# ultralytics/yolov3

Measured on AMD Instinct MI355X. Metric: images/sec (640x640) inference+NMS, higher is better.
Workload: dtype f16; 1 GPU; yolov3 inference 640x640 batch=32/GPU fp16 nc=80 + NMS(conf 0.001, iou 0.6, multi_label, max_det 300) [BASELINE configs[1]]; global_batch=32, parallelism=replicas x1 (no data-path collective)

## Files before the change

include/yolov3_hip.h:

```cpp
#ifndef YOLOV3_HIP_H
#define YOLOV3_HIP_H

#include <stddef.h>
#include <stdint.h>

#ifdef __cplusplus
extern "C" {
#endif

#define Y3_ABI_VERSION 6

typedef enum { Y3_F16 = 0, Y3_BF16 = 1, Y3_F32 = 2, Y3_U8 = 3 } y3_dtype;
typedef enum { Y3_ACT_NONE = 0, Y3_ACT_SILU = 1 } y3_act;
typedef enum { Y3_ALGO_AUTO = 0, Y3_ALGO_MFMA = 1, Y3_ALGO_DIRECT = 2 } y3_algo;

typedef struct {
    void* data;
    int32_t n, h, w, c;
    int32_t pitch;
} y3_tensor;

typedef struct {
    int32_t dtype;
    int32_t ksize;
// ... 27 lines not shown
int y3_conv2d_fwd_variant(const y3_conv_desc* desc, const y3_tensor* x, const y3_tensor* y, int32_t has_residual,
                          size_t workspace_bytes, char* name, size_t name_capacity);
int y3_conv_v10_tiles(const y3_conv_desc* desc, const y3_tensor* x, const y3_tensor* y, size_t workspace_bytes, int32_t* records,
                      int64_t capacity, int64_t* n_tiles, int32_t* column_blocks, int32_t* group_blocks);
int64_t y3_conv2d_fwd_bnin_rows(const y3_conv_desc* desc, const y3_tensor* u_in, const y3_tensor* y_in, const y3_tensor* y, int32_t has_shortcut);
int y3_conv2d_fwd_bnin_stats(const y3_conv_desc* desc, const y3_tensor* u_in, const float* in_scale, const float* in_shift, int32_t in_act,
                             const y3_tensor* in_shortcut , const y3_tensor* y_in, const void* packed_filter, const float* bias, const y3_tensor* y,
                             float* stat_rows, int64_t capacity_rows, int64_t* n_rows, void* stream);
int y3_conv_last_variant(char* name, size_t name_cap);

size_t y3_packed_filter_stem_elems(int32_t cout);
int y3_pack_filter_stem(const float* w_oihw, int32_t cout_src, int32_t cin_src, int32_t cout, int32_t dtype, void* packed, void* stream);
int y3_stem_conv_fwd(const void* x_nchw, int32_t src_dtype, int32_t n, int32_t cin, int32_t h, int32_t w, float divisor, const void* packed,
                     const float* bias, int32_t dtype, int32_t act, const y3_tensor* y, void* stream);
int64_t y3_stem_conv_stats_rows(int32_t n, int32_t h, int32_t w);
int y3_stem_conv_fwd_stats(const void* x_nchw, int32_t src_dtype, int32_t n, int32_t cin, int32_t h, int32_t w, float divisor, const void* packed,
                           const float* bias, int32_t dtype, int32_t act, const y3_tensor* y, float* stat_rows, int64_t capacity_rows, int64_t* n_rows,
                           void* stream);
int y3_stem_pair_fwd(const void* x_nchw, int32_t src_dtype, int32_t n, int32_t cin, int32_t h, int32_t w, float divisor,
                     const void* packed0, const float* bias0, int32_t act0, const void* packed1, const float* bias1, int32_t act1,
                     int32_t dtype, const y3_tensor* y, void* stream);
int y3_bneck_pair_fwd(const y3_tensor* x, const void* packed1, const float* bias1, int32_t act1, const void* packed2, const float* bias2,
                      int32_t act2, int32_t add_residual, int32_t dtype, const y3_tensor* y, void* stream);

int y3_nchw_to_nhwc(const void* src, int32_t src_dtype, int32_t n, int32_t c, int32_t h, int32_t w, float divisor,
                    int32_t out_dtype, const y3_tensor* out, void* stream);
int y3_nhwc_to_nchw(const y3_tensor* src, int32_t dtype, void* dst, void* stream);

int y3_maxpool2d(const y3_tensor* x, const y3_tensor* y, int32_t dtype, int32_t k, int32_t stride, int32_t pad,
                 int32_t zpad_r, int32_t zpad_b, void* stream);
int y3_spp_pyramid(const y3_tensor* x, const y3_tensor* y3c , int32_t dtype,
                   void* stream);
int y3_upsample2x(const y3_tensor* x, const y3_tensor* y, int32_t dtype, void* stream);
int y3_copy_slice(const y3_tensor* x, const y3_tensor* y, int32_t dtype, void* stream);

int y3_detect_decode(const y3_tensor* head, int32_t dtype, int32_t na, int32_t no, const float* anchors_px,
                     float stride, void* raw, void* z, int64_t row_offset, int64_t total_rows, void* stream);
int y3_detect_decode_levels(const y3_tensor* heads, int32_t n_levels, int32_t dtype, int32_t na, int32_t no,
                            const float* anchors_px, const float* strides, void* const* raws, void* z,
                            const int64_t* row_offsets, int64_t total_rows, void* stream);

typedef struct {
    double iou_thres;
    float conf_thres;
    int32_t multi_label, agnostic;
    int32_t max_det, max_nms;
// ... 269 lines not shown
```

yolov3_amd/csrc/api.cpp:

```cpp
#include <atomic>
#include <mutex>
#include <stdarg.h>
#include <stdio.h>
#include <stdlib.h>
#include <string.h>

#include "../../include/yolov3_hip.h"
#include "y3_knobs.h"

static thread_local char g_err[512] = "";

void y3_set_error(const char* fmt, ...) {
    va_list ap;
    va_start(ap, fmt);
    vsnprintf(g_err, sizeof(g_err), fmt, ap);
    va_end(ap);
}

extern "C" const char* y3_last_error(void) { return g_err; }
extern "C" int y3_abi_version(void) { return Y3_ABI_VERSION; }

namespace {
struct Knob {
    const char* name;
    long long def;
};
const Knob kKnobs[] = {
    {"conv", 0}, {"conv_ahead", 3}, {"bn_nt_bytes", 64ll << 20},
    {"wgrad", 0}, {"wgrad_xcd", 2}, {"dgrad_quad", 1}, {"spp_direct", 0}, {"wgrad_strip", 1}, {"conv_strip", 1},
    {"conv_v10", 1}, {"v10_mp", 0}, {"v10_blocks", 0}, {"v10_half", 2}, {"v10_ksplit", 1}, {"v10_slices", 0},
    {"v10_group", 1}, {"tile_xcd", 1}, {"conv_1x1s", 1}, {"wgrad_patch", 1}, {"wgrad_blocks", 512}, {"nms_sort", 1},
    {"decode_tile", 1}, {"nms_head", 1216},
};
constexpr int kCount = (int)(sizeof(kKnobs) / sizeof(kKnobs[0]));
static_assert(kCount == Y3K_COUNT, "kKnobs and y3_knob_id (y3_common.h) list the same knobs in the same order");
std::atomic<long long> g_val[kCount];
std::once_flag g_once;

int knob_index(const char* key) {
    for (int i = 0; i < kCount; ++i)
        if (key && !strcmp(key, kKnobs[i].name)) return i;
    return -1;
}
void load_defaults() {
    for (int i = 0; i < kCount; ++i) g_val[i].store(kKnobs[i].def, std::memory_order_relaxed);
    const char* e = getenv("Y3_TUNE");
    if (!e) return;
    char buf[512];
    strncpy(buf, e, sizeof(buf) - 1);
    buf[sizeof(buf) - 1] = 0;
    for (char* tok = strtok(buf, ",;"); tok; tok = strtok(nullptr, ",;")) {
        char* eq = strchr(tok, '=');
        if (!eq) continue;
        *eq = 0;
        const int i = knob_index(tok);
// ... 37 lines not shown
```

yolov3_amd/csrc/stem.hip:

```cpp
#include "../../include/yolov3_hip.h"
#include "y3_common.h"

#include <hip/hip_runtime.h>
#include <stdint.h>
#include <type_traits>
#include <utility>

namespace {

struct StemArgs {
    const void* x;
    const void* w;
    const float* bias;
    void* y;
    int N, Cin, H, W;
    int ypitch, Cout;
    int act;
    int tiles_w, tiles_h;
    float divisor;
    float* stats;
};

constexpr int TR = 8, TW = 64;
constexpr int PR = TR + 2;
// ... 128 lines not shown
        }
        __builtin_amdgcn_fence(__ATOMIC_RELEASE, "wavefront");
        __builtin_amdgcn_wave_barrier();
    }
    if (want_stats) {
#pragma unroll
        for (int off = CH; off < 64; off <<= 1)
#pragma unroll
            for (int q = 0; q < 8; ++q) { st0[q] += __shfl_xor(st0[q], off, 64); st1[q] += __shfl_xor(st1[q], off, 64); }
        __syncthreads();
        float* red = (float*)patch;
        if (rp == 0) {
#pragma unroll
            for (int q = 0; q < 8; ++q) { red[(wv * CH + ch) * 16 + 2 * q] = st0[q]; red[(wv * CH + ch) * 16 + 2 * q + 1] = st1[q]; }
        }
        __syncthreads();
        if (tid < CH * 16 && (tid >> 4) * 8 + 8 <= p.Cout) {
            const float v = red[tid] + red[CH * 16 + tid] + red[2 * CH * 16 + tid] + red[3 * CH * 16 + tid];
            p.stats[(long long)blockIdx.x * p.Cout * 2 + tid] = v;
        }
    }
}

struct PairArgs {
    const void* x;
    const void* w0;
    const float* b0;
    const void* w1;
    const float* b1;
    void* y;
    int N, Cin, H, W, Ho, Wo, ypitch, act0, act1, kpad1;
    int tiles_w, tiles_h, n_tiles;
    int xcd;
    float divisor;
#ifdef Y3_TIMELINE
    unsigned long long* tl;
#endif
};
#ifdef Y3_TIMELINE
static unsigned long long* g_pair_tl = nullptr;
#define SP_T(i) do { asm volatile("s_waitcnt lgkmcnt(0)" ::: "memory"); const unsigned long long t_ = __builtin_amdgcn_s_memtime(); asm volatile("s_waitcnt lgkmcnt(0)" ::: "memory"); tsum[i] += t_ - tprev; tprev = t_; } while (0)
#else
#define SP_T(i) do { } while (0)
#endif
constexpr int QR = 4, QW = 32;
constexpr int R0 = 2 * QR + 1, C0 = 2 * QW + 1;
constexpr int XR = R0 + 2, XW = C0 + 3;
constexpr int L0E = C0 / 2 + 1, L0ROW = C0 * 64;

template <typename T, typename S>
__global__ __launch_bounds__(256, 2) void stem_pair_kernel(const PairArgs p) {
    typedef typename Mfma16<T>::frag frag;
    typedef T vec4 __attribute__((ext_vector_type(4)));
    typedef unsigned u32x4 __attribute__((ext_vector_type(4)));
    constexpr int PATCH_BYTES = XR * XW * 8, SLICE_BYTES = 4 * 32 * 64;
// ... 20 lines not shown
#pragma unroll
    for (int j = 0; j < NPX; ++j) {
        const int e = tid + j * 256;
        const int pr = e / XW;
        prc[j] = e < XR * XW ? (pr << 8) | (e - pr * XW) : -1;
    }
    constexpr int NT0 = (R0 * C0 + 31) / 32, NJ0 = (NT0 + 3) / 4;
    int l0rd[NJ0], l0wr[NJ0], l0rc[NJ0];
#pragma unroll
    for (int j = 0; j < NJ0; ++j) {
        int q = (wv + 4 * j) * 32 + frow;
        const bool live = q < R0 * C0;
        if (!live) q = R0 * C0 - 1;
        const int r = q / C0, c = q - r * C0, ci = c >> 1;
        l0rd[j] = (r * XW + c + 2 * fk) * 8;
        l0wr[j] = live ? r * L0ROW + ((c & 1) ? L0E * 64 : 0) + ci * 64 + ((fk ^ ((ci >> 2) & 3)) << 4) : -1;
        l0rc[j] = (r << 8) | c;
    }
    const int hw = p.H * p.W;

    T* __restrict__ yg = (T*)p.y;
    S raw[NPX][4];
    bool rin[NPX];
    auto fetch = [&](int tile) {
        int b = tile;
        const int tw = b % p.tiles_w; b /= p.tiles_w;
        const int th = b % p.tiles_h;
        const int n = b / p.tiles_h;
        const int gh0 = 2 * th * QR - 2, gw0 = 2 * tw * QW - 2;
        const S* __restrict__ xs = (const S*)p.x + (long long)n * p.Cin * hw;
#pragma unroll
        for (int j = 0; j < NPX; ++j) {
            const int gh = gh0 + (prc[j] >> 8), gw = gw0 + (prc[j] & 255);
            rin[j] = prc[j] >= 0 && (unsigned)gh < (unsigned)p.H && (unsigned)gw < (unsigned)p.W;
            if (rin[j]) {
                const unsigned o = (unsigned)(gh * p.W + gw);
#pragma unroll
                for (int c = 0; c < 4; ++c)
                    if (c < p.Cin) raw[j][c] = xs[o + (unsigned)(c * hw)];
            }
        }
    };
    const bool plain = std::is_same<S, T>::value && p.divisor == 1.0f;
    auto stash = [&]() {
#pragma unroll
        for (int j = 0; j < NPX; ++j) {
            const int e = tid + j * 256;
            if (e < XR * XW) {
                vec4 v = {(T)0.0f, (T)0.0f, (T)0.0f, (T)0.0f};
                if (rin[j]) {
                    bool done = false;
                    if constexpr (std::is_same<S, T>::value) {
                        if (plain) {
#pragma unroll
                            for (int c = 0; c < 4; ++c)
                                if (c < p.Cin) v[c] = raw[j][c];
                            done = true;
                        }
                    }
                    if (!done) {
#pragma unroll
                        for (int c = 0; c < 4; ++c)
                            if (c < p.Cin) v[c] = from_f32<T>(src_f32<S>(raw[j][c]) / p.divisor);
                    }
                }
                *(vec4*)(scratch + e * 8) = v;
            }
        }
    };
    const int first = p.xcd ? xcd_remap((int)blockIdx.x, (int)gridDim.x) : (int)blockIdx.x;
    if (first < p.n_tiles) fetch(first);
#ifdef Y3_TIMELINE
    unsigned long long tsum[8] = {0, 0, 0, 0, 0, 0, 0, 0};
    unsigned long long tprev = __builtin_amdgcn_s_memtime();
#endif
    for (int tile = first; tile < p.n_tiles; tile += gridDim.x) {
        int b = tile;
        const int tw = b % p.tiles_w; b /= p.tiles_w;
        const int th = b % p.tiles_h;
        const int n = b / p.tiles_h;
        const int oh0 = th * QR, ow0 = tw * QW;
        const int gh0 = 2 * oh0 - 1, gw0 = 2 * ow0 - 1;
        const bool border = gh0 < 0 || gw0 < 0 || gh0 + R0 > p.H || gw0 + C0 > p.W;

        stash();
        SP_T(0);
        __syncthreads();
        SP_T(1);

#pragma unroll
        for (int j = 0; j < NJ0; ++j) {
            if (wv + 4 * j >= NT0) break;
            f32x16 acc;
#pragma unroll
            for (int g = 0; g < 4; ++g)
#pragma unroll
                for (int e = 0; e < 4; ++e) acc[4 * g + e] = cb0[8 * g + 4 * fk + e];
#pragma unroll
            for (int kh = 0; kh < 3; ++kh) {
                const unsigned char* src = scratch + l0rd[j] + kh * (XW * 8);
                typedef unsigned long long u64x2 __attribute__((ext_vector_type(2)));
                u64x2 rw;
                rw[0] = *(const unsigned long long*)src;
                rw[1] = *(const unsigned long long*)(src + 8);
                acc = Mfma16<T>::run(*(const frag*)(cw0 + ((frow * 3 + kh) * 16 + fk * 8) * 2), __builtin_bit_cast(frag, rw), acc);
            }
            if (p.act0 == Y3_ACT_SILU) silu_vec<f32x16, 16>(acc);
            bool keep = l0wr[j] >= 0;
            bool inside = true;
            if (border) inside = (unsigned)(gh0 + (l0rc[j] >> 8)) < (unsigned)p.H && (unsigned)(gw0 + (l0rc[j] & 255)) < (unsigned)p.W;
#pragma unroll
            for (int gp = 0; gp < 2; ++gp) {
                u32x4 ov;
#pragma unroll
                for (int h = 0; h < 2; ++h) {
                    const unsigned a = pack2<T>(acc[8 * gp + 2 * h], acc[8 * gp + 2 * h + 1]);
                    const unsigned b = pack2<T>(acc[8 * gp + 4 + 2 * h], acc[8 * gp + 4 + 2 * h + 1]);
                    const auto sw = __builtin_amdgcn_permlane32_swap(a, b, false, false);
                    ov[h] = inside ? (unsigned)sw[0] : 0u;
                    ov[2 + h] = inside ? (unsigned)sw[1] : 0u;
                }
                if (keep) *(u32x4*)(l0buf + (l0wr[j] ^ (gp << 5))) = ov;
            }
        }
        SP_T(2);
        __syncthreads();
        SP_T(3);
        if (tile + (int)gridDim.x < p.n_tiles) fetch(tile + gridDim.x);

        f32x16 acc1[2];
#pragma unroll
        for (int b2 = 0; b2 < 2; ++b2)
#pragma unroll
            for (int g = 0; g < 4; ++g)
#pragma unroll
                for (int e = 0; e < 4; ++e) acc1[b2][4 * g + e] = cb1[wc * 32 + 8 * g + 4 * fk + e];
#pragma unroll
        for (int tap = 0; tap < 9; ++tap) {
            const int kh = tap / 3, kw = tap - 3 * (tap / 3);
#pragma unroll
            for (int ks = 0; ks < 2; ++ks)
#pragma unroll
                for (int b2 = 0; b2 < 2; ++b2) {
                    const int lr = 2 * wp + b2;
                    const int ci = frow + (kw >> 1);
                    const frag bf = *(const frag*)(l0buf + (2 * lr + kh) * L0ROW + ((kw & 1) ? L0E * 64 : 0) + ci * 64 + (((ks * 2 + fk) ^ ((ci >> 2) & 3)) << 4));
                    acc1[b2] = Mfma16<T>::run(a1f[tap * 2 + ks], bf, acc1[b2]);
                }
        }
        SP_T(4);
        unsigned char* wl = scratch + wv * (32 * 64);
// ... 32 lines not shown
            __builtin_amdgcn_fence(__ATOMIC_RELEASE, "wavefront");
            __builtin_amdgcn_wave_barrier();
        }
        SP_T(5);
        __syncthreads();
        SP_T(6);
    }
#ifdef Y3_TIMELINE
    if (p.tl && blockIdx.x < 64 && lane == 0) {
#pragma unroll
        for (int i = 0; i < 8; ++i) p.tl[(blockIdx.x * 4 + wv) * 8 + i] = tsum[i];
    }
#endif
}

struct BneckArgs {
    const void* x;
    const void* w1;
    const float* b1;
    const void* w2;
    const float* b2;
    void* y;
    int N, H, W, xpitch, ypitch, act1, act2, add, kpad1, kpad2;
    int tiles_w, tiles_h, n_tiles;
    int xcd;
    unsigned x_bytes;
};
constexpr int BC = 32, RC = BC + 2;
constexpr int bneck_rows(int c) { return c == 64 ? 8 : 4; }
constexpr int L1PITCH = 40;

template <typename F, int... Is> Y3_DEV void sfor_impl(F&& f, std::integer_sequence<int, Is...>) { (f(std::integral_constant<int, Is>{}), ...); }
template <int N, typename F> Y3_DEV void sfor(F&& f) { sfor_impl(f, std::make_integer_sequence<int, N>{}); }

template <typename T, int C>
__global__ __launch_bounds__(C * 4, C == 64 ? 2 : 1) void bneck_pair_kernel(const BneckArgs p) {
    typedef typename Mfma16<T>::frag frag;
    typedef unsigned u32x4 __attribute__((ext_vector_type(4)));
    typedef __attribute__((address_space(3))) void* lds_ptr_t;
    constexpr int BR = bneck_rows(C), RW = BR / 2;
    constexpr int RR = BR + 2, RPX = RR * RC;
    constexpr int NT1 = (RPX + 31) / 32;
    constexpr int CM = C / 2;
    constexpr int FT = C / 32;
    constexpr int NWV = 2 * FT;
    constexpr int XB = C * 2, XCHK = XB / 16;
    constexpr int LB = CM * 2, LCHK = LB / 16;
    constexpr int K1S = C / 16, M1 = CM / 32;
    constexpr int KT = CM / 16;
    constexpr int K2S = 9 * KT;
    constexpr int XPIECES = (RPX * XCHK + 63) / 64;
    constexpr int XJ = (XPIECES + NWV - 1) / NWV;
    constexpr int NJ1 = (NT1 + NWV - 1) / NWV;
    constexpr int QSTEP = 32 * NWV;
    constexpr int XKS = XCHK == 8 ? 1 : 0;
    constexpr int LKS = LCHK == 4 ? 2 : 1;
    __shared__ __attribute__((aligned(16))) unsigned char xbuf[XPIECES * 1024];
    __shared__ __attribute__((aligned(16))) unsigned char l1buf[RR * L1PITCH * LB];
    __shared__ __attribute__((aligned(16))) unsigned char slices[NWV * 32 * 64];
    __shared__ __attribute__((aligned(16))) float cb1[CM], cb2[C];
    constexpr bool W1_LDS = C == 128;
    __shared__ __attribute__((aligned(16))) unsigned char cw1[W1_LDS ? CM * C * 2 : 16];

    const int tid = threadIdx.x, lane = tid & 63;
    const int wv = __builtin_amdgcn_readfirstlane(tid >> 6);
    const int frow = lane & 31, fk = lane >> 5;
    const int wc = wv >> 1, wp = wv & 1;

    if (tid < CM / 4) ((f32x4*)cb1)[tid] = ((const f32x4*)p.b1)[tid];
    else if (tid < CM / 4 + C / 4) ((f32x4*)cb2)[tid - CM / 4] = ((const f32x4*)p.b2)[tid - CM / 4];
    if constexpr (W1_LDS) {
        for (int i = tid; i < CM * XCHK; i += 64 * NWV) {
            const int r = i / XCHK, c = i % XCHK;
            *(u32x4*)(cw1 + r * XB + ((c ^ (r & 15)) << 4)) = *(const u32x4*)((const T*)p.w1 + (long long)r * p.kpad1 + c * 8);
        }
    }
    frag a2f[K2S];
#pragma unroll
    for (int t = 0; t < K2S; ++t) a2f[t] = *(const frag*)((const T*)p.w2 + (long long)(wc * 32 + frow) * p.kpad2 + t * 16 + fk * 8);

    const auto rs_x = __builtin_amdgcn_make_buffer_rsrc((void*)p.x, 0, (int)p.x_bytes, 0x00020000);
    const int c1q0 = 32 * wv + frow;
    const int c1r0 = c1q0 / RC, c1c0 = c1q0 - c1r0 * RC;
    const int c1rd0 = c1q0 * XB + ((fk ^ ((c1q0 >> XKS) & (XCHK - 1))) << 4);
    int c2rd[3];
#pragma unroll
    for (int kw = 0; kw < 3; ++kw) c2rd[kw] = (frow + kw) * LB + ((fk ^ (((frow + kw) >> LKS) & (LCHK - 1))) << 4);

    T* __restrict__ yg = (T*)p.y;
    auto fetch = [&](int tile) {
        int b = tile;
        const int tw = b % p.tiles_w; b /= p.tiles_w;
        const int th = b % p.tiles_h;
        const int n = b / p.tiles_h;
        const int gh0 = th * BR - 1, gw0 = tw * BC - 1;
        int lane_f = lane;
        asm volatile("" : "+v"(lane_f));
        const int xq0 = (64 / XCHK) * wv + lane_f / XCHK;
        const unsigned xsrc = (unsigned)(((lane_f % XCHK) ^ ((xq0 >> XKS) & (XCHK - 1))) * 16);
        int r = 0, c = xq0;
#pragma unroll
        for (int j = 0; j < XJ; ++j) {
            if (wv + NWV * j >= XPIECES) break;
            const int gh = gh0 + r, gw = gw0 + c;
            const bool ok = xq0 + 32 * j < RPX && (unsigned)gh < (unsigned)p.H && (unsigned)gw < (unsigned)p.W;
            const unsigned off = ok ? (unsigned)(((n * p.H + gh) * p.W + gw) * p.xpitch) * 2u + xsrc : 0xffffffffu;
            const unsigned ldsa = __builtin_amdgcn_readfirstlane((unsigned)(uintptr_t)(lds_ptr_t)xbuf + (unsigned)((wv + NWV * j) * 1024));
            asm volatile("s_mov_b32 m0, %0\n\ts_nop 0\n\tbuffer_load_dwordx4 %1, %2, 0 offen lds" : : "s"(ldsa), "v"(off), "s"(rs_x) : "memory");
            c += 32;
            if (c >= RC) { c -= RC; r += 1; }
        }
    };
    const int first = p.xcd ? xcd_remap((int)blockIdx.x, (int)gridDim.x) : (int)blockIdx.x;
    if (first < p.n_tiles) fetch(first);
    for (int tile = first; tile < p.n_tiles; tile += gridDim.x) {
        int b = tile;
        const int tw = b % p.tiles_w; b /= p.tiles_w;
        const int th = b % p.tiles_h;
        const int n = b / p.tiles_h;
        const int oh0 = th * BR, ow0 = tw * BC;
        const int gh0 = oh0 - 1, gw0 = ow0 - 1;
        const bool border = gh0 < 0 || gw0 < 0 || gh0 + RR > p.H || gw0 + RC > p.W;

        frag a1g[W1_LDS ? 1 : K1S * M1];
        if constexpr (!W1_LDS) {
#pragma unroll
            for (int ks = 0; ks < K1S; ++ks)
#pragma unroll
                for (int m = 0; m < M1; ++m) a1g[ks * M1 + m] = *(const frag*)((const T*)p.w1 + (long long)(m * 32 + frow) * p.kpad1 + ks * 16 + fk * 8);
        }
        __builtin_amdgcn_s_waitcnt(0x0F70);
        __syncthreads();

        {
            f32x16 acc[NJ1][M1];
#pragma unroll
            for (int j = 0; j < NJ1; ++j)
#pragma unroll
                for (int m = 0; m < M1; ++m)
#pragma unroll
                    for (int g = 0; g < 4; ++g)
#pragma unroll
                        for (int e = 0; e < 4; ++e) acc[j][m][4 * g + e] = cb1[m * 32 + 8 * g + 4 * fk + e];
#pragma unroll
            for (int ks = 0; ks < K1S; ++ks) {
                frag af[M1];
#pragma unroll
                for (int m = 0; m < M1; ++m) {
                    if constexpr (W1_LDS) af[m] = *(const frag*)(cw1 + (m * 32 + frow) * XB + (((2 * ks + fk) ^ (frow & 15)) << 4));
                    else af[m] = a1g[ks * M1 + m];
                }
#pragma unroll
                for (int j = 0; j < NJ1; ++j) {
                    if (wv + NWV * j >= NT1) break;
                    const frag bf = *(const frag*)(xbuf + ((c1rd0 + j * (QSTEP * XB)) ^ (ks << 5)));
#pragma unroll
                    for (int m = 0; m < M1; ++m) acc[j][m] = Mfma16<T>::run(af[m], bf, acc[j][m]);
                }
            }
            int r1 = c1r0, c1 = c1c0;
#pragma unroll
            for (int j = 0; j < NJ1; ++j) {
                if (wv + NWV * j >= NT1) break;
                const bool live = c1q0 + QSTEP * j < RPX;
                bool inside = true;
                if (border) inside = (unsigned)(gh0 + r1) < (unsigned)p.H && (unsigned)(gw0 + c1) < (unsigned)p.W;
                const int wr = (r1 * L1PITCH + c1) * LB + ((fk ^ ((c1 >> LKS) & (LCHK - 1)) ^ ((r1 & 1) * (LCHK / 2))) << 4);
#pragma unroll
                for (int m = 0; m < M1; ++m) {
                    if (p.act1 == Y3_ACT_SILU) silu_vec<f32x16, 16>(acc[j][m]);
#pragma unroll
                    for (int gp = 0; gp < 2; ++gp) {
                        u32x4 ov;
#pragma unroll
                        for (int h = 0; h < 2; ++h) {
                            const auto sw = __builtin_amdgcn_permlane32_swap(pack2<T>(acc[j][m][8 * gp + 2 * h], acc[j][m][8 * gp + 2 * h + 1]),
                                                                             pack2<T>(acc[j][m][8 * gp + 4 + 2 * h], acc[j][m][8 * gp + 4 + 2 * h + 1]), false, false);
                            ov[h] = inside ? (unsigned)sw[0] : 0u;
                            ov[2 + h] = inside ? (unsigned)sw[1] : 0u;
                        }
                        if (live) *(u32x4*)(l1buf + (wr ^ ((m * 4 + gp * 2) << 4))) = ov;
                    }
                    __builtin_amdgcn_sched_barrier(0);
                }
                c1 += QSTEP % RC;
                r1 += QSTEP / RC;
                if (c1 >= RC) { c1 -= RC; r1 += 1; }
            }
        }
        u32x4 xres[2 * RW];
        if (p.add) {
            int lane_r = lane;
            asm volatile("" : "+v"(lane_r));
            const int rp_r = lane_r >> 2, lc = wc * 4 + (lane_r & 3);
#pragma unroll
            for (int b2 = 0; b2 < RW; ++b2)
#pragma unroll
                for (int i = 0; i < 2; ++i) {
                    const int q = (RW * wp + b2 + 1) * RC + (i * 16 + rp_r + 1);
                    xres[b2 * 2 + i] = *(const u32x4*)(xbuf + q * XB + ((lc ^ ((q >> XKS) & (XCHK - 1))) << 4));
                }
        }
        __syncthreads();
        {
            int nt = tile + (int)gridDim.x;
            asm volatile("" : "+s"(nt));
            if (nt < p.n_tiles) fetch(nt);
        }
        f32x16 acc2[RW];
#pragma unroll
        for (int b2 = 0; b2 < RW; ++b2)
#pragma unroll
            for (int g = 0; g < 4; ++g)
#pragma unroll
                for (int e = 0; e < 4; ++e) acc2[b2][4 * g + e] = cb2[wc * 32 + 8 * g + 4 * fk + e];
        const unsigned char* l1w = l1buf + (RW * wp) * (L1PITCH * LB);
        auto rd = [&](auto step_c, frag (&bf)[RW]) {
            constexpr int tap = decltype(step_c)::value / KT, ks = decltype(step_c)::value % KT, kh = tap / 3, kw = tap - 3 * (tap / 3);
#pragma unroll
            for (int b2 = 0; b2 < RW; ++b2) {
                const int rr = b2 + kh;
                bf[b2] = *(const frag*)(l1w + rr * (L1PITCH * LB) + (c2rd[kw] ^ (((2 * ks) ^ ((rr & 1) * (LCHK / 2))) << 4)));
            }
        };
        auto mm = [&](auto step_c, const frag (&bf)[RW]) {
#pragma unroll
            for (int b2 = 0; b2 < RW; ++b2) acc2[b2] = Mfma16<T>::run(a2f[decltype(step_c)::value], bf[b2], acc2[b2]);
        };
        frag bA[RW], bB[RW];
        rd(std::integral_constant<int, 0>{}, bA);
// ... 107 lines not shown
    hipStream_t st = (hipStream_t)stream;
    switch (dtype) {
        case Y3_F16: return dispatch_src<f16_t>(a, src_dtype, st);
        case Y3_BF16: return dispatch_src<bf16_t>(a, src_dtype, st);
    }
    Y3_FAIL("%s: f16/bf16 compute only", who);
}

extern "C" int y3_stem_conv_fwd(const void* x_nchw, int32_t src_dtype, int32_t n, int32_t cin, int32_t h, int32_t w, float divisor, const void* packed,
                                const float* bias, int32_t dtype, int32_t act, const y3_tensor* y, void* stream) {
    return stem_conv_impl(x_nchw, src_dtype, n, cin, h, w, divisor, packed, bias, dtype, act, y, nullptr, 0, nullptr, stream, "y3_stem_conv_fwd");
}

extern "C" int64_t y3_stem_conv_stats_rows(int32_t n, int32_t h, int32_t w) { return (int64_t)((w + TW - 1) / TW) * ((h + TR - 1) / TR) * n; }

extern "C" int y3_stem_conv_fwd_stats(const void* x_nchw, int32_t src_dtype, int32_t n, int32_t cin, int32_t h, int32_t w, float divisor, const void* packed,
                                      const float* bias, int32_t dtype, int32_t act, const y3_tensor* y, float* stat_rows, int64_t capacity_rows, int64_t* n_rows,
                                      void* stream) {
    if (!stat_rows || !n_rows) Y3_FAIL("y3_stem_conv_fwd_stats: null statistics buffer");
    return stem_conv_impl(x_nchw, src_dtype, n, cin, h, w, divisor, packed, bias, dtype, act, y, stat_rows, capacity_rows, n_rows, stream, "y3_stem_conv_fwd_stats");
}

namespace {
template <typename T> int dispatch_pair(const PairArgs& a, int sdt, long long tiles, hipStream_t st) {
    const int cap = 2 * y3_cu_count();
    const int blocks = tiles < cap ? (int)tiles : cap;
    switch (sdt) {
        case Y3_F16: hipLaunchKernelGGL((stem_pair_kernel<T, f16_t>), dim3((unsigned)blocks), dim3(256), 0, st, a); break;
        case Y3_BF16: hipLaunchKernelGGL((stem_pair_kernel<T, bf16_t>), dim3((unsigned)blocks), dim3(256), 0, st, a); break;
        case Y3_F32: hipLaunchKernelGGL((stem_pair_kernel<T, float>), dim3((unsigned)blocks), dim3(256), 0, st, a); break;
        case Y3_U8: hipLaunchKernelGGL((stem_pair_kernel<T, unsigned char>), dim3((unsigned)blocks), dim3(256), 0, st, a); break;
        default: Y3_FAIL("y3_stem_pair_fwd: bad source dtype %d", sdt);
    }
    Y3_CHECK_LAUNCH();
    return 0;
}
}

#ifdef Y3_TIMELINE
extern "C" void y3_debug_pair_timeline(void* buf) { g_pair_tl = (unsigned long long*)buf; }
#endif

extern "C" int y3_stem_pair_fwd(const void* x_nchw, int32_t src_dtype, int32_t n, int32_t cin, int32_t h, int32_t w, float divisor, const void* packed0, const float* bias0,
                                int32_t act0, const void* packed1, const float* bias1, int32_t act1, int32_t dtype, const y3_tensor* y, void* stream) {
    if (!x_nchw || !packed0 || !bias0 || !packed1 || !bias1 || !y || !y->data) Y3_FAIL("y3_stem_pair_fwd: null argument");
    if (cin < 1 || cin > 4) Y3_FAIL("y3_stem_pair_fwd: %d input channels (1..4 supported)", cin);
    const int Ho = (h - 1) / 2 + 1, Wo = (w - 1) / 2 + 1;
    if (y->n != n || y->h != Ho || y->w != Wo || y->c != 64) Y3_FAIL("y3_stem_pair_fwd: output must be (%d,%d,%d,64)", n, Ho, Wo);
    if ((y->pitch % 8) || ((uintptr_t)y->data & 15) || ((uintptr_t)packed0 & 15) || ((uintptr_t)packed1 & 15) || ((uintptr_t)bias0 & 15) || ((uintptr_t)bias1 & 15))
        Y3_FAIL("y3_stem_pair_fwd: 16-byte aligned views");
    if (!(divisor > 0.0f)) Y3_FAIL("y3_stem_pair_fwd: divisor must be positive");
    if ((long long)n * h * w > 0x7fffffffLL) Y3_FAIL("y3_stem_pair_fwd: too many pixels");
    PairArgs a;
    a.x = x_nchw; a.w0 = packed0; a.b0 = bias0; a.w1 = packed1; a.b1 = bias1; a.y = y->data;
    a.N = n; a.Cin = cin; a.H = h; a.W = w; a.Ho = Ho; a.Wo = Wo; a.ypitch = y->pitch; a.act0 = act0; a.act1 = act1;
    a.kpad1 = y3_filter_kpad(32, 3);
    a.tiles_w = (Wo + QW - 1) / QW; a.tiles_h = (Ho + QR - 1) / QR;
    const long long tiles = (long long)a.tiles_w * a.tiles_h * n;
    if (tiles > 0x7fffffffLL) Y3_FAIL("y3_stem_pair_fwd: too many tiles");
    a.n_tiles = (int)tiles;
    a.xcd = y3_knob(Y3K_TILE_XCD) != 0;
    a.divisor = divisor;
#ifdef Y3_TIMELINE
    a.tl = g_pair_tl;
#endif
    hipStream_t st = (hipStream_t)stream;
    switch (dtype) {
        case Y3_F16: return dispatch_pair<f16_t>(a, src_dtype, tiles, st);
        case Y3_BF16: return dispatch_pair<bf16_t>(a, src_dtype, tiles, st);
    }
    Y3_FAIL("y3_stem_pair_fwd: f16/bf16 compute only");
}

extern "C" int y3_bneck_pair_fwd(const y3_tensor* x, const void* packed1, const float* bias1, int32_t act1, const void* packed2, const float* bias2, int32_t act2,
                                 int32_t add_residual, int32_t dtype, const y3_tensor* y, void* stream) {
    if (!x || !x->data || !packed1 || !bias1 || !packed2 || !bias2 || !y || !y->data) Y3_FAIL("y3_bneck_pair_fwd: null argument");
    const int c = x->c;
    if ((c != 64 && c != 128) || y->c != c) Y3_FAIL("y3_bneck_pair_fwd: Bottleneck(64, 64) or Bottleneck(128, 128) (cv1 C -> C/2 1x1, cv2 C/2 -> C 3x3), got %d -> %d channels", x->c, y->c);
    if (y->n != x->n || y->h != x->h || y->w != x->w) Y3_FAIL("y3_bneck_pair_fwd: output shape");
    if ((x->pitch % 8) || (y->pitch % 8) || ((uintptr_t)x->data & 15) || ((uintptr_t)y->data & 15) || ((uintptr_t)packed1 & 15) || ((uintptr_t)packed2 & 15) ||
        ((uintptr_t)bias1 & 15) || ((uintptr_t)bias2 & 15))
        Y3_FAIL("y3_bneck_pair_fwd: 16-byte aligned views");
    if (x->data == y->data) Y3_FAIL("y3_bneck_pair_fwd: in-place operation is not supported (tiles read their neighbours' input)");
    BneckArgs a;
    a.x = x->data; a.w1 = packed1; a.b1 = bias1; a.w2 = packed2; a.b2 = bias2; a.y = y->data;
    a.N = x->n; a.H = x->h; a.W = x->w; a.xpitch = x->pitch; a.ypitch = y->pitch; a.act1 = act1; a.act2 = act2; a.add = add_residual ? 1 : 0;
    a.kpad1 = y3_filter_kpad(c, 1); a.kpad2 = y3_filter_kpad(c / 2, 3);
    a.tiles_w = (x->w + BC - 1) / BC; a.tiles_h = (x->h + bneck_rows(c) - 1) / bneck_rows(c);
    const long long tiles = (long long)a.tiles_w * a.tiles_h * x->n;
    if (tiles > 0x7fffffffLL || (long long)x->n * x->h * x->w > 0x7fffffffLL) Y3_FAIL("y3_bneck_pair_fwd: too many pixels");
    a.n_tiles = (int)tiles;
    a.xcd = y3_knob(Y3K_TILE_XCD) != 0;
    const long long xb = (((long long)x->n * x->h * x->w - 1) * x->pitch + x->c) * 2;
    if (xb >= 0x7fffffffLL) Y3_FAIL("y3_bneck_pair_fwd: input beyond the 2 GiB reach of a buffer descriptor (split the batch)");
    a.x_bytes = (unsigned)xb;
    const int cap = (c == 64 ? 2 : 1) * y3_cu_count();
    const int blocks = tiles < cap ? (int)tiles : cap;
    hipStream_t st = (hipStream_t)stream;
    if (dtype != Y3_F16 && dtype != Y3_BF16) Y3_FAIL("y3_bneck_pair_fwd: f16/bf16 only");
    if (c == 64) {
        if (dtype == Y3_F16) hipLaunchKernelGGL((bneck_pair_kernel<f16_t, 64>), dim3((unsigned)blocks), dim3(256), 0, st, a);
        else hipLaunchKernelGGL((bneck_pair_kernel<bf16_t, 64>), dim3((unsigned)blocks), dim3(256), 0, st, a);
    } else {
        if (dtype == Y3_F16) hipLaunchKernelGGL((bneck_pair_kernel<f16_t, 128>), dim3((unsigned)blocks), dim3(512), 0, st, a);
        else hipLaunchKernelGGL((bneck_pair_kernel<bf16_t, 128>), dim3((unsigned)blocks), dim3(512), 0, st, a);
    }
    Y3_CHECK_LAUNCH();
    return 0;
}
```

yolov3_amd/csrc/y3_common.h:

```cpp
#pragma once
#include <hip/hip_runtime.h>
#include <stdint.h>
#include <stdio.h>
#include <string.h>

#include "../../include/yolov3_hip.h"

#define Y3_DEV __device__ __forceinline__

typedef _Float16 f16_t;
typedef __bf16 bf16_t;
typedef float f32x4 __attribute__((ext_vector_type(4)));
typedef float f32x8 __attribute__((ext_vector_type(8)));
typedef float f32x16 __attribute__((ext_vector_type(16)));
typedef _Float16 f16x8 __attribute__((ext_vector_type(8)));
typedef __bf16 bf16x8 __attribute__((ext_vector_type(8)));

void y3_set_error(const char* fmt, ...);
#define Y3_FAIL(...)               \
    do {                           \
        y3_set_error(__VA_ARGS__); \
        return -1;                 \
    } while (0)
#define Y3_CHECK_LAUNCH()                                                     \
    do {                                                                      \
        hipError_t e_ = hipGetLastError();                                    \
        if (e_ != hipSuccess) Y3_FAIL("%s:%d launch failed: %s", __FILE__, __LINE__, hipGetErrorString(e_)); \
    } while (0)

#define Y3_HIP(call)                                                                          \
    do {                                                                                      \
        hipError_t e_ = (call);                                                               \
        if (e_ != hipSuccess) Y3_FAIL("%s:%d %s failed: %s", __FILE__, __LINE__, #call, hipGetErrorString(e_)); \
    } while (0)

#include "y3_knobs.h"

Y3_DEV int xcd_remap(int b, int nb) {
    const int xcd = b & 7, i = b >> 3;
    const int q = nb >> 3, r = nb & 7;
    const int base = xcd < r ? xcd * (q + 1) : r * (q + 1) + (xcd - r) * q;
    return base + i;
}

template <typename T> Y3_DEV float to_f32(T v);
template <> Y3_DEV float to_f32<f16_t>(f16_t v) { return (float)v; }
template <> Y3_DEV float to_f32<bf16_t>(bf16_t v) { return (float)v; }
template <> Y3_DEV float to_f32<float>(float v) { return v; }
template <typename T> Y3_DEV T from_f32(float v);
template <> Y3_DEV f16_t from_f32<f16_t>(float v) { return (f16_t)v; }
template <> Y3_DEV bf16_t from_f32<bf16_t>(float v) { return (bf16_t)v; }
template <> Y3_DEV float from_f32<float>(float v) { return v; }

typedef float f32x2 __attribute__((ext_vector_type(2)));
template <typename T> Y3_DEV unsigned pack2(float a, float b);
template <> Y3_DEV unsigned pack2<f16_t>(float a, float b) {
    typedef _Float16 h2 __attribute__((ext_vector_type(2)));
    const f32x2 v = {a, b};
    return __builtin_bit_cast(unsigned, __builtin_convertvector(v, h2));
}
template <> Y3_DEV unsigned pack2<bf16_t>(float a, float b) {
// ... 69 lines not shown
```

yolov3_amd/csrc/y3_knobs.h:

```cpp
#pragma once
enum y3_knob_id {
    Y3K_CONV = 0,
    Y3K_CONV_AHEAD,
    Y3K_BN_NT_BYTES,
    Y3K_WGRAD,
    Y3K_WGRAD_XCD,
    Y3K_DGRAD_QUAD,
    Y3K_SPP_DIRECT,
    Y3K_WGRAD_STRIP,
    Y3K_CONV_STRIP,
    Y3K_CONV_V10,
    Y3K_V10_MP,
    Y3K_V10_BLOCKS,
    Y3K_V10_HALF,
    Y3K_V10_KSPLIT,
    Y3K_V10_SLICES,
    Y3K_V10_GROUP,
    Y3K_TILE_XCD,
    Y3K_CONV_1X1S,
    Y3K_WGRAD_PATCH,
    Y3K_WGRAD_BLOCKS,
    Y3K_NMS_SORT,
    Y3K_DECODE_TILE,
    Y3K_NMS_HEAD,
    Y3K_COUNT
};
long long y3_knob(int id);
```

Before: 5456 images/sec.

## Walk pair-kernel tiles in vertical runs and carry halo rows in LDS

Stem-pair and bottleneck-pair fused kernels now walk consecutive vertical tiles in runs of length L (default 5) per block. The first-stage halo rows already computed for the previous tile are kept in LDS and copied into place, so the overlapping rows are neither refetched nor recomputed. This removes redundant conv work and global loads at tile seams, but adds register staging of the carried rows and more complex tile scheduling that may unbalance load across blocks. The block cap for the 128-channel bottleneck changes from 1x to 1x CU and stem stays 2x, and a host-side helper that lists tiles per block is added.

```diff
diff --git a/include/yolov3_hip.h b/include/yolov3_hip.h
--- a/include/yolov3_hip.h
+++ b/include/yolov3_hip.h
@@ -73,6 +73,8 @@
                      int32_t dtype, const y3_tensor* y, void* stream);
 int y3_bneck_pair_fwd(const y3_tensor* x, const void* packed1, const float* bias1, int32_t act1, const void* packed2, const float* bias2,
                       int32_t act2, int32_t add_residual, int32_t dtype, const y3_tensor* y, void* stream);
+int y3_pair_tiles(int32_t channels, int32_t n, int32_t h, int32_t w, int32_t block, int32_t* records, int64_t capacity, int64_t* n_tiles,
+                  int32_t* n_blocks);
 
 int y3_nchw_to_nhwc(const void* src, int32_t src_dtype, int32_t n, int32_t c, int32_t h, int32_t w, float divisor,
                     int32_t out_dtype, const y3_tensor* out, void* stream);
diff --git a/yolov3_amd/csrc/api.cpp b/yolov3_amd/csrc/api.cpp
--- a/yolov3_amd/csrc/api.cpp
+++ b/yolov3_amd/csrc/api.cpp
@@ -30,7 +30,7 @@
     {"wgrad", 0}, {"wgrad_xcd", 2}, {"dgrad_quad", 1}, {"spp_direct", 0}, {"wgrad_strip", 1}, {"conv_strip", 1},
     {"conv_v10", 1}, {"v10_mp", 0}, {"v10_blocks", 0}, {"v10_half", 2}, {"v10_ksplit", 1}, {"v10_slices", 0},
     {"v10_group", 1}, {"tile_xcd", 1}, {"conv_1x1s", 1}, {"wgrad_patch", 1}, {"wgrad_blocks", 512}, {"nms_sort", 1},
-    {"decode_tile", 1}, {"nms_head", 1216},
+    {"decode_tile", 1}, {"nms_head", 1216}, {"pair_run", 5}, {"pair_blocks", 0},
 };
 constexpr int kCount = (int)(sizeof(kKnobs) / sizeof(kKnobs[0]));
 static_assert(kCount == Y3K_COUNT, "kKnobs and y3_knob_id (y3_common.h) list the same knobs in the same order");
diff --git a/yolov3_amd/csrc/stem.hip b/yolov3_amd/csrc/stem.hip
--- a/yolov3_amd/csrc/stem.hip
+++ b/yolov3_amd/csrc/stem.hip
@@ -174,6 +174,28 @@
     }
 }
 
+struct PairGeom {
+    int tiles_w, tiles_h;
+    int L, runs_h, n_runs;
+};
+struct PairTile {
+    int n, th, tw;
+};
+__host__ __device__ inline PairTile pair_tile(const PairGeom& g, int run, int t) {
+    PairTile o;
+    int b = run;
+    o.tw = b % g.tiles_w; b /= g.tiles_w;
+    o.th = (b % g.runs_h) * g.L + t;
+    o.n = b / g.runs_h;
+    return o;
+}
+__host__ __device__ inline bool pair_next(const PairGeom& g, int grid, int& run, int& t) {
+    const int th = (run / g.tiles_w) % g.runs_h * g.L + t + 1;
+    if (t + 1 < g.L && th < g.tiles_h) ++t;
+    else { t = 0; run += grid; }
+    return run < g.n_runs;
+}
+
 struct PairArgs {
     const void* x;
     const void* w0;
@@ -182,7 +204,7 @@
     const float* b1;
     void* y;
     int N, Cin, H, W, Ho, Wo, ypitch, act0, act1, kpad1;
-    int tiles_w, tiles_h, n_tiles;
+    PairGeom g;
     int xcd;
     float divisor;
 #ifdef Y3_TIMELINE
@@ -249,17 +271,13 @@
     T* __restrict__ yg = (T*)p.y;
     S raw[NPX][4];
     bool rin[NPX];
-    auto fetch = [&](int tile) {
-        int b = tile;
-        const int tw = b % p.tiles_w; b /= p.tiles_w;
-        const int th = b % p.tiles_h;
-        const int n = b / p.tiles_h;
-        const int gh0 = 2 * th * QR - 2, gw0 = 2 * tw * QW - 2;
-        const S* __restrict__ xs = (const S*)p.x + (long long)n * p.Cin * hw;
+    auto fetch = [&](const PairTile ft, int skip) {
+        const int gh0 = 2 * ft.th * QR - 2 + skip, gw0 = 2 * ft.tw * QW - 2;
+        const S* __restrict__ xs = (const S*)p.x + (long long)ft.n * p.Cin * hw;
 #pragma unroll
         for (int j = 0; j < NPX; ++j) {
             const int gh = gh0 + (prc[j] >> 8), gw = gw0 + (prc[j] & 255);
-            rin[j] = prc[j] >= 0 && (unsigned)gh < (unsigned)p.H && (unsigned)gw < (unsigned)p.W;
+            rin[j] = prc[j] >= 0 && (prc[j] >> 8) < XR - skip && (unsigned)gh < (unsigned)p.H && (unsigned)gw < (unsigned)p.W;
             if (rin[j]) {
                 const unsigned o = (unsigned)(gh * p.W + gw);
 #pragma unroll
@@ -295,29 +313,43 @@
             }
         }
     };
-    const int first = p.xcd ? xcd_remap((int)blockIdx.x, (int)gridDim.x) : (int)blockIdx.x;
-    if (first < p.n_tiles) fetch(first);
+    int run = p.xcd ? xcd_remap((int)blockIdx.x, (int)gridDim.x) : (int)blockIdx.x, t = 0;
+    bool more = run < p.g.n_runs;
+    if (more) fetch(pair_tile(p.g, run, 0), 0);
 #ifdef Y3_TIMELINE
     unsigned long long tsum[8] = {0, 0, 0, 0, 0, 0, 0, 0};
     unsigned long long tprev = __builtin_amdgcn_s_memtime();
 #endif
-    for (int tile = first; tile < p.n_tiles; tile += gridDim.x) {
-        int b = tile;
-        const int tw = b % p.tiles_w; b /= p.tiles_w;
-        const int th = b % p.tiles_h;
-        const int n = b / p.tiles_h;
-        const int oh0 = th * QR, ow0 = tw * QW;
+    constexpr int NT0C = ((R0 - 1) * C0 + 31) / 32;
+    constexpr int CARRY = L0ROW / 16, NCR = (CARRY + 255) / 256;
+    while (more) {
+        const PairTile ct = pair_tile(p.g, run, t);
+        const int skip = t ? 1 : 0;
+        const int n = ct.n;
+        const int oh0 = ct.th * QR, ow0 = ct.tw * QW;
         const int gh0 = 2 * oh0 - 1, gw0 = 2 * ow0 - 1;
         const bool border = gh0 < 0 || gw0 < 0 || gh0 + R0 > p.H || gw0 + C0 > p.W;
 
+        u32x4 cr[NCR];
+        if (skip) {
+#pragma unroll
+            for (int i = 0; i < NCR; ++i)
+                if (tid + i * 256 < CARRY) cr[i] = *(const u32x4*)(l0buf + (R0 - 1) * L0ROW + (tid + i * 256) * 16);
+        }
         stash();
         SP_T(0);
         __syncthreads();
         SP_T(1);
-
+        if (skip) {
+#pragma unroll
+            for (int i = 0; i < NCR; ++i)
+                if (tid + i * 256 < CARRY) *(u32x4*)(l0buf + (tid + i * 256) * 16) = cr[i];
+        }
+
+        const int nt0 = skip ? NT0C : NT0;
 #pragma unroll
         for (int j = 0; j < NJ0; ++j) {
-            if (wv + 4 * j >= NT0) break;
+            if (wv + 4 * j >= nt0) break;
             f32x16 acc;
 #pragma unroll
             for (int g = 0; g < 4; ++g)
@@ -333,9 +365,10 @@
                 acc = Mfma16<T>::run(*(const frag*)(cw0 + ((frow * 3 + kh) * 16 + fk * 8) * 2), __builtin_bit_cast(frag, rw), acc);
             }
             if (p.act0 == Y3_ACT_SILU) silu_vec<f32x16, 16>(acc);
-            bool keep = l0wr[j] >= 0;
+            const int rr = (l0rc[j] >> 8) + skip;
+            bool keep = l0wr[j] >= 0 && rr < R0;
             bool inside = true;
-            if (border) inside = (unsigned)(gh0 + (l0rc[j] >> 8)) < (unsigned)p.H && (unsigned)(gw0 + (l0rc[j] & 255)) < (unsigned)p.W;
+            if (border) inside = (unsigned)(gh0 + rr) < (unsigned)p.H && (unsigned)(gw0 + (l0rc[j] & 255)) < (unsigned)p.W;
 #pragma unroll
             for (int gp = 0; gp < 2; ++gp) {
                 u32x4 ov;
@@ -347,13 +380,14 @@
                     ov[h] = inside ? (unsigned)sw[0] : 0u;
                     ov[2 + h] = inside ? (unsigned)sw[1] : 0u;
                 }
-                if (keep) *(u32x4*)(l0buf + (l0wr[j] ^ (gp << 5))) = ov;
+                if (keep) *(u32x4*)(l0buf + skip * L0ROW + (l0wr[j] ^ (gp << 5))) = ov;
             }
         }
         SP_T(2);
         __syncthreads();
         SP_T(3);
-        if (tile + (int)gridDim.x < p.n_tiles) fetch(tile + gridDim.x);
+        more = pair_next(p.g, (int)gridDim.x, run, t);
+        if (more) fetch(pair_tile(p.g, run, t), t ? 1 : 0);
 
         f32x16 acc1[2];
 #pragma unroll
@@ -432,7 +466,7 @@
     const float* b2;
     void* y;
     int N, H, W, xpitch, ypitch, act1, act2, add, kpad1, kpad2;
-    int tiles_w, tiles_h, n_tiles;
+    PairGeom g;
     int xcd;
     unsigned x_bytes;
 };
@@ -451,6 +485,7 @@
     constexpr int BR = bneck_rows(C), RW = BR / 2;
     constexpr int RR = BR + 2, RPX = RR * RC;
     constexpr int NT1 = (RPX + 31) / 32;
+    constexpr int CPX = BR * RC, NT1C = (CPX + 31) / 32;
     constexpr int CM = C / 2;
     constexpr int FT = C / 32;
     constexpr int NWV = 2 * FT;
@@ -492,18 +527,15 @@
     const auto rs_x = __builtin_amdgcn_make_buffer_rsrc((void*)p.x, 0, (int)p.x_bytes, 0x00020000);
     const int c1q0 = 32 * wv + frow;
     const int c1r0 = c1q0 / RC, c1c0 = c1q0 - c1r0 * RC;
-    const int c1rd0 = c1q0 * XB + ((fk ^ ((c1q0 >> XKS) & (XCHK - 1))) << 4);
     int c2rd[3];
 #pragma unroll
     for (int kw = 0; kw < 3; ++kw) c2rd[kw] = (frow + kw) * LB + ((fk ^ (((frow + kw) >> LKS) & (LCHK - 1))) << 4);
 
     T* __restrict__ yg = (T*)p.y;
-    auto fetch = [&](int tile) {
-        int b = tile;
-        const int tw = b % p.tiles_w; b /= p.tiles_w;
-        const int th = b % p.tiles_h;
-        const int n = b / p.tiles_h;
-        const int gh0 = th * BR - 1, gw0 = tw * BC - 1;
+    auto fetch = [&](const PairTile ft, int skip) {
+        const int n = ft.n;
+        const int gh0 = ft.th * BR - 1 + skip, gw0 = ft.tw * BC - 1;
+        const int npx = (RR - skip) * RC;
         int lane_f = lane;
         asm volatile("" : "+v"(lane_f));
         const int xq0 = (64 / XCHK) * wv + lane_f / XCHK;
@@ -511,9 +543,9 @@
         int r = 0, c = xq0;
 #pragma unroll
         for (int j = 0; j < XJ; ++j) {
-            if (wv + NWV * j >= XPIECES) break;
+            if ((wv + NWV * j) * (64 / XCHK) >= npx) break;
             const int gh = gh0 + r, gw = gw0 + c;
-            const bool ok = xq0 + 32 * j < RPX && (unsigned)gh < (unsigned)p.H && (unsigned)gw < (unsigned)p.W;
+            const bool ok = xq0 + 32 * j < npx && (unsigned)gh < (unsigned)p.H && (unsigned)gw < (unsigned)p.W;
             const unsigned off = ok ? (unsigned)(((n * p.H + gh) * p.W + gw) * p.xpitch) * 2u + xsrc : 0xffffffffu;
             const unsigned ldsa = __builtin_amdgcn_readfirstlane((unsigned)(uintptr_t)(lds_ptr_t)xbuf + (unsigned)((wv + NWV * j) * 1024));
             asm volatile("s_mov_b32 m0, %0\n\ts_nop 0\n\tbuffer_load_dwordx4 %1, %2, 0 offen lds" : : "s"(ldsa), "v"(off), "s"(rs_x) : "memory");
@@ -521,16 +553,18 @@
             if (c >= RC) { c -= RC; r += 1; }
         }
     };
-    const int first = p.xcd ? xcd_remap((int)blockIdx.x, (int)gridDim.x) : (int)blockIdx.x;
-    if (first < p.n_tiles) fetch(first);
-    for (int tile = first; tile < p.n_tiles; tile += gridDim.x) {
-        int b = tile;
-        const int tw = b % p.tiles_w; b /= p.tiles_w;
-        const int th = b % p.tiles_h;
-        const int n = b / p.tiles_h;
-        const int oh0 = th * BR, ow0 = tw * BC;
+    int run = p.xcd ? xcd_remap((int)blockIdx.x, (int)gridDim.x) : (int)blockIdx.x, t = 0;
+    bool more = run < p.g.n_runs;
+    if (more) fetch(pair_tile(p.g, run, 0), 0);
+    constexpr int CARRY = 2 * RC * LCHK, NCR = (CARRY + 64 * NWV - 1) / (64 * NWV);
+    while (more) {
+        const PairTile ct = pair_tile(p.g, run, t);
+        const bool cont = t != 0;
+        const int n = ct.n;
+        const int oh0 = ct.th * BR, ow0 = ct.tw * BC;
         const int gh0 = oh0 - 1, gw0 = ow0 - 1;
         const bool border = gh0 < 0 || gw0 < 0 || gh0 + RR > p.H || gw0 + RC > p.W;
+        const int xskip = cont ? RC : 0;
 
         frag a1g[W1_LDS ? 1 : K1S * M1];
         if constexpr (!W1_LDS) {
@@ -539,10 +573,28 @@
 #pragma unroll
                 for (int m = 0; m < M1; ++m) a1g[ks * M1 + m] = *(const frag*)((const T*)p.w1 + (long long)(m * 32 + frow) * p.kpad1 + ks * 16 + fk * 8);
         }
+        u32x4 cr[NCR];
+        int cro[NCR];
+        if (cont) {
+#pragma unroll
+            for (int i = 0; i < NCR; ++i) {
+                const int e = tid + i * (64 * NWV), px = e / LCHK, r = px / RC;
+                cro[i] = e < CARRY ? (r * L1PITCH + px - r * RC) * LB + (e % LCHK) * 16 : -1;
+                if (cro[i] >= 0) cr[i] = *(const u32x4*)(l1buf + BR * L1PITCH * LB + cro[i]);
+            }
+        }
         __builtin_amdgcn_s_waitcnt(0x0F70);
         __syncthreads();
+        if (cont) {
+#pragma unroll
+            for (int i = 0; i < NCR; ++i)
+                if (cro[i] >= 0) *(u32x4*)(l1buf + cro[i]) = cr[i];
+        }
 
         {
+            const int nt1 = cont ? NT1C : NT1;
+            const int c1qx = c1q0 + (cont ? RC : 0);
+            const int c1rd0 = c1qx * XB + ((fk ^ ((c1qx >> XKS) & (XCHK - 1))) << 4);
             f32x16 acc[NJ1][M1];
 #pragma unroll
             for (int j = 0; j < NJ1; ++j)
@@ -562,17 +614,17 @@
                 }
 #pragma unroll
                 for (int j = 0; j < NJ1; ++j) {
-                    if (wv + NWV * j >= NT1) break;
+                    if (wv + NWV * j >= nt1) break;
                     const frag bf = *(const frag*)(xbuf + ((c1rd0 + j * (QSTEP * XB)) ^ (ks << 5)));
 #pragma unroll
                     for (int m = 0; m < M1; ++m) acc[j][m] = Mfma16<T>::run(af[m], bf, acc[j][m]);
                 }
             }
-            int r1 = c1r0, c1 = c1c0;
+            int r1 = c1r0 + (cont ? 2 : 0), c1 = c1c0;
 #pragma unroll
             for (int j = 0; j < NJ1; ++j) {
-                if (wv + NWV * j >= NT1) break;
-                const bool live = c1q0 + QSTEP * j < RPX;
+                if (wv + NWV * j >= nt1) break;
+                const bool live = c1q0 + QSTEP * j < (cont ? CPX : RPX);
                 bool inside = true;
                 if (border) inside = (unsigned)(gh0 + r1) < (unsigned)p.H && (unsigned)(gw0 + c1) < (unsigned)p.W;
                 const int wr = (r1 * L1PITCH + c1) * LB + ((fk ^ ((c1 >> LKS) & (LCHK - 1)) ^ ((r1 & 1) * (LCHK / 2))) << 4);
@@ -607,15 +659,16 @@
             for (int b2 = 0; b2 < RW; ++b2)
 #pragma unroll
                 for (int i = 0; i < 2; ++i) {
-                    const int q = (RW * wp + b2 + 1) * RC + (i * 16 + rp_r + 1);
+                    const int q = (RW * wp + b2 + 1) * RC + (i * 16 + rp_r + 1) - xskip;
                     xres[b2 * 2 + i] = *(const u32x4*)(xbuf + q * XB + ((lc ^ ((q >> XKS) & (XCHK - 1))) << 4));
                 }
         }
         __syncthreads();
         {
-            int nt = tile + (int)gridDim.x;
-            asm volatile("" : "+s"(nt));
-            if (nt < p.n_tiles) fetch(nt);
+            more = pair_next(p.g, (int)gridDim.x, run, t);
+            int nr = run;
+            asm volatile("" : "+s"(nr));
+            if (more) fetch(pair_tile(p.g, nr, t), t ? 1 : 0);
         }
         f32x16 acc2[RW];
 #pragma unroll
@@ -769,9 +822,22 @@
 }
 
 namespace {
-template <typename T> int dispatch_pair(const PairArgs& a, int sdt, long long tiles, hipStream_t st) {
-    const int cap = 2 * y3_cu_count();
-    const int blocks = tiles < cap ? (int)tiles : cap;
+int pair_plan(int c, int n, int h, int w, PairGeom* g, int* blocks, const char* who) {
+    const int tr = c ? bneck_rows(c) : QR, tc = c ? BC : QW;
+    g->tiles_w = (w + tc - 1) / tc; g->tiles_h = (h + tr - 1) / tr;
+    const long long want = y3_knob(Y3K_PAIR_RUN);
+    g->L = want < 1 ? 1 : want > g->tiles_h ? g->tiles_h : (int)want;
+    g->runs_h = (g->tiles_h + g->L - 1) / g->L;
+    const long long tiles = (long long)g->tiles_w * g->tiles_h * n, runs = (long long)g->tiles_w * g->runs_h * n;
+    const long long forced = y3_knob(Y3K_PAIR_BLOCKS);
+    const long long cap = forced > 0 ? (forced < 65536 ? forced : 65536) : (long long)(c == 128 ? 1 : 2) * y3_cu_count();
+    if (tiles < 1 || tiles > 0x7fffffffLL - cap) Y3_FAIL("%s: no tiles, or too many", who);
+    g->n_runs = (int)runs;
+    *blocks = runs < cap ? (int)runs : (int)cap;
+    return 0;
+}
+
+template <typename T> int dispatch_pair(const PairArgs& a, int sdt, int blocks, hipStream_t st) {
     switch (sdt) {
         case Y3_F16: hipLaunchKernelGGL((stem_pair_kernel<T, f16_t>), dim3((unsigned)blocks), dim3(256), 0, st, a); break;
         case Y3_BF16: hipLaunchKernelGGL((stem_pair_kernel<T, bf16_t>), dim3((unsigned)blocks), dim3(256), 0, st, a); break;
@@ -802,10 +868,8 @@
     a.x = x_nchw; a.w0 = packed0; a.b0 = bias0; a.w1 = packed1; a.b1 = bias1; a.y = y->data;
     a.N = n; a.Cin = cin; a.H = h; a.W = w; a.Ho = Ho; a.Wo = Wo; a.ypitch = y->pitch; a.act0 = act0; a.act1 = act1;
     a.kpad1 = y3_filter_kpad(32, 3);
-    a.tiles_w = (Wo + QW - 1) / QW; a.tiles_h = (Ho + QR - 1) / QR;
-    const long long tiles = (long long)a.tiles_w * a.tiles_h * n;
-    if (tiles > 0x7fffffffLL) Y3_FAIL("y3_stem_pair_fwd: too many tiles");
-    a.n_tiles = (int)tiles;
+    int blocks = 0;
+    if (pair_plan(0, n, Ho, Wo, &a.g, &blocks, "y3_stem_pair_fwd")) return -1;
     a.xcd = y3_knob(Y3K_TILE_XCD) != 0;
     a.divisor = divisor;
 #ifdef Y3_TIMELINE
@@ -813,8 +877,8 @@
 #endif
     hipStream_t st = (hipStream_t)stream;
     switch (dtype) {
-        case Y3_F16: return dispatch_pair<f16_t>(a, src_dtype, tiles, st);
-        case Y3_BF16: return dispatch_pair<bf16_t>(a, src_dtype, tiles, st);
+        case Y3_F16: return dispatch_pair<f16_t>(a, src_dtype, blocks, st);
+        case Y3_BF16: return dispatch_pair<bf16_t>(a, src_dtype, blocks, st);
     }
     Y3_FAIL("y3_stem_pair_fwd: f16/bf16 compute only");
 }
@@ -833,16 +897,13 @@
     a.x = x->data; a.w1 = packed1; a.b1 = bias1; a.w2 = packed2; a.b2 = bias2; a.y = y->data;
     a.N = x->n; a.H = x->h; a.W = x->w; a.xpitch = x->pitch; a.ypitch = y->pitch; a.act1 = act1; a.act2 = act2; a.add = add_residual ? 1 : 0;
     a.kpad1 = y3_filter_kpad(c, 1); a.kpad2 = y3_filter_kpad(c / 2, 3);
-    a.tiles_w = (x->w + BC - 1) / BC; a.tiles_h = (x->h + bneck_rows(c) - 1) / bneck_rows(c);
-    const long long tiles = (long long)a.tiles_w * a.tiles_h * x->n;
-    if (tiles > 0x7fffffffLL || (long long)x->n * x->h * x->w > 0x7fffffffLL) Y3_FAIL("y3_bneck_pair_fwd: too many pixels");
-    a.n_tiles = (int)tiles;
+    if ((long long)x->n * x->h * x->w > 0x7fffffffLL) Y3_FAIL("y3_bneck_pair_fwd: too many pixels");
+    int blocks = 0;
+    if (pair_plan(c, x->n, x->h, x->w, &a.g, &blocks, "y3_bneck_pair_fwd")) return -1;
     a.xcd = y3_knob(Y3K_TILE_XCD) != 0;
     const long long xb = (((long long)x->n * x->h * x->w - 1) * x->pitch + x->c) * 2;
     if (xb >= 0x7fffffffLL) Y3_FAIL("y3_bneck_pair_fwd: input beyond the 2 GiB reach of a buffer descriptor (split the batch)");
     a.x_bytes = (unsigned)xb;
-    const int cap = (c == 64 ? 2 : 1) * y3_cu_count();
-    const int blocks = tiles < cap ? (int)tiles : cap;
     hipStream_t st = (hipStream_t)stream;
     if (dtype != Y3_F16 && dtype != Y3_BF16) Y3_FAIL("y3_bneck_pair_fwd: f16/bf16 only");
     if (c == 64) {
@@ -855,3 +916,23 @@
     Y3_CHECK_LAUNCH();
     return 0;
 }
+
+extern "C" int y3_pair_tiles(int32_t channels, int32_t n, int32_t h, int32_t w, int32_t block, int32_t* records, int64_t capacity, int64_t* n_tiles, int32_t* n_blocks) {
+    if (!n_tiles || !n_blocks) Y3_FAIL("y3_pair_tiles: null argument");
+    if ((channels != 0 && channels != 64 && channels != 128) || n < 1 || h < 1 || w < 1) Y3_FAIL("y3_pair_tiles: channels 0 (stem_pair) / 64 / 128 (bneck_pair), a non-empty batch");
+    PairGeom g;
+    int blocks = 0;
+    if (pair_plan(channels, n, channels ? h : (h - 1) / 2 + 1, channels ? w : (w - 1) / 2 + 1, &g, &blocks, "y3_pair_tiles")) return -1;
+    *n_blocks = blocks;
+    if (block < 0 || block >= blocks) Y3_FAIL("y3_pair_tiles: block %d of %d", block, blocks);
+    int64_t cnt = 0;
+    int run = y3_knob(Y3K_TILE_XCD) != 0 ? xcd_remap(block, blocks) : block, t = 0;
+    for (bool more = run < g.n_runs; more; more = pair_next(g, blocks, run, t), ++cnt) {
+        if (!records || cnt >= capacity) continue;
+        const PairTile ct = pair_tile(g, run, t);
+        int32_t* r = records + cnt * 4;
+        r[0] = ct.n; r[1] = ct.th; r[2] = ct.tw; r[3] = t == 0;
+    }
+    *n_tiles = cnt;
+    return 0;
+}
diff --git a/yolov3_amd/csrc/y3_common.h b/yolov3_amd/csrc/y3_common.h
--- a/yolov3_amd/csrc/y3_common.h
+++ b/yolov3_amd/csrc/y3_common.h
@@ -36,7 +36,7 @@
 
 #include "y3_knobs.h"
 
-Y3_DEV int xcd_remap(int b, int nb) {
+__host__ Y3_DEV int xcd_remap(int b, int nb) {
     const int xcd = b & 7, i = b >> 3;
     const int q = nb >> 3, r = nb & 7;
     const int base = xcd < r ? xcd * (q + 1) : r * (q + 1) + (xcd - r) * q;
diff --git a/yolov3_amd/csrc/y3_knobs.h b/yolov3_amd/csrc/y3_knobs.h
--- a/yolov3_amd/csrc/y3_knobs.h
+++ b/yolov3_amd/csrc/y3_knobs.h
@@ -23,6 +23,8 @@
     Y3K_NMS_SORT,
     Y3K_DECODE_TILE,
     Y3K_NMS_HEAD,
+    Y3K_PAIR_RUN,
+    Y3K_PAIR_BLOCKS,
     Y3K_COUNT
 };
 long long y3_knob(int id);
```

Result: slower. 5397 images/sec (-1.1%).
